# Ledicia/Molecular-Dynamics-Simulation---Lennard-Jones-monoatomic-fluid

Measured on AMD Instinct MI355X. Metric: md_steps_per_sec_n262144_fp64, higher is better.
Workload: dtype f64

## Files before the change

molecular-dynamics-simulation---lennard-jones-monoatomic-fluid_amd/csrc/ljmd_common.cpp:

```cpp
#include "ljmd_common.h"
#include "ljmd_internal.h"

#include <algorithm>
#include <cstdio>
#include <cstring>
#include <limits>

namespace ljmdh {

using namespace ljmdk;

thread_local std::string g_last_error = "";

int failv(std::string *handle_err, int code, const char *fmt, va_list ap)
{
    char buf[512];
    vsnprintf(buf, sizeof buf, fmt, ap);
    g_last_error = buf;
    if (handle_err) *handle_err = buf;
    return code;
}

int check_sim_params(const char *who, int n, double box_length, double dt, double rc)
{
// ... 42 lines not shown
Knobs read_knobs()
{
    auto flag = [](const char *name, bool dflt) { return env_int(name, dflt ? 1 : 0) != 0; };
    auto is = [](const char *name, const char *value) {
        const char *v = std::getenv(name);
        return v && std::strcmp(v, value) == 0;
    };
    auto opt_int = [](const char *name) -> std::optional<int> {
        const char *v = std::getenv(name);
        if (v && *v) return std::atoi(v);
        return std::nullopt;
    };
    Knobs k;
    k.sort = flag("LJMD_SORT", k.sort);
    k.force_generic = flag("LJMD_FORCE_GENERIC", k.force_generic);
    k.force_collectives = flag("LJMD_FORCE_COLLECTIVES", k.force_collectives);
    k.fuse = flag("LJMD_FUSE", k.fuse);
    k.fuse_tail = flag("LJMD_FUSE_TAIL", k.fuse_tail);
    k.fuse_defer_record = flag("LJMD_FUSE_DEFER_RECORD", k.fuse_defer_record);
    k.xcd_remap = std::max(0, env_int("LJMD_N3_XCD_REMAP", k.xcd_remap));
    k.inject_failure_at_step = env_int("LJMD_INJECT_FAILURE_AT_STEP", k.inject_failure_at_step);
    k.exchange_alltoall = is("LJMD_FORCE_EXCHANGE", "alltoall");
    k.resort_every = opt_int("LJMD_RESORT_EVERY");
    k.n3_row_tiles = env_int("LJMD_N3_ROW_TILES", k.n3_row_tiles);
    k.n3_wg_waves = env_int("LJMD_N3_WG_WAVES", k.n3_wg_waves);
    k.slab_budget_gb = std::max(1, env_int("LJMD_SLAB_BUDGET_GB", k.slab_budget_gb));
    k.n3_both_ties = flag("LJMD_N3_BOTH_TIES", k.n3_both_ties);
    k.n3_min_n = env_int("LJMD_N3_MIN_N", k.n3_min_n);
    k.n3 = flag("LJMD_N3", k.n3);
    k.n3_target_waves = opt_int("LJMD_N3_TARGET_WAVES");
    k.n3_clusters = flag("LJMD_N3_CLUSTERS", k.n3_clusters);
    k.n3_pertile = flag("LJMD_N3_PERTILE", k.n3_pertile);
    k.reduce_split = opt_int("LJMD_REDUCE_SPLIT");
    if (k.reduce_split) k.reduce_split = std::max(0, *k.reduce_split);
    k.walk_chunk = opt_int("LJMD_WALK_CHUNK");
    k.vanhove_chunk = opt_int("LJMD_VANHOVE_CHUNK");
    k.fp32_far_stream = flag("LJMD_FP32_FAR_STREAM", k.fp32_far_stream);
    k.fp32_vfar = flag("LJMD_FP32_VFAR", k.fp32_vfar);
    {
        const char *rs = std::getenv("LJMD_FP32_SPLIT");
        if (rs && *rs) k.fp32_split = std::max(0.0, std::atof(rs));
    }
    k.overlap_exchange = flag("LJMD_OVERLAP_EXCHANGE", k.overlap_exchange);
    k.migrate_blocks = is("LJMD_MIGRATE_DEAL", "blocks");
    {
        const char *xm = std::getenv("LJMD_MULTI_EXCHANGE");
// ... 80 lines not shown
```

molecular-dynamics-simulation---lennard-jones-monoatomic-fluid_amd/csrc/ljmd_common.h:

```cpp
#ifndef LJMD_COMMON_H
#define LJMD_COMMON_H

#include "ljmd.h"

#include <hip/hip_runtime.h>

#include <cstdarg>
#include <cstddef>
#include <cstdint>
#include <cstdlib>
#include <optional>
#include <string>

namespace ljmdh {

extern thread_local std::string g_last_error;

constexpr double kPi = 3.1415926535897932384626433832795;

int failv(std::string *handle_err, int code, const char *fmt, va_list ap);

inline int fail(std::nullptr_t, int code, const char *fmt, ...)
{
    va_list ap;
// ... 49 lines not shown
struct SimParams {
    double L = 0, invL = 0, volume = 0, rc = 0, rc2 = 0, dt = 0, dt_half = 0, dt_sq_half = 0;
    double tail_e = 0, tail_d = 0, tail_dd = 0;
};
SimParams derive_params(int n, double box_length, double dt, double rc);

void scalars_from_sums(double s12, double s6, double kx, double ky, double kz, double te, double td, double tdd,
                       double *epot, double *ekin, double *d_epot, double *dd_epot);

void scalars_from_exact_sums(const uint64_t (&ordered)[5][3], double te, double td, double tdd, bool have_e, bool have_k,
                             double *epot, double *ekin, double *d_epot, double *dd_epot);

struct Knobs {
    bool sort = true;
    bool force_generic = false;
    bool force_collectives = false;
    bool fuse = true;
    bool fuse_tail = true;
    bool fuse_defer_record = true;
    int xcd_remap = 4;
    int inject_failure_at_step = -1;
    bool exchange_alltoall = false;
    std::optional<int> resort_every;
    int n3_row_tiles = 0;
    int n3_wg_waves = 0;
    int slab_budget_gb = 64;
    bool n3_both_ties = true;
    int n3_min_n = 4096;
    bool n3 = true;
    std::optional<int> n3_target_waves;
    bool n3_clusters = true;
    bool n3_pertile = true;
    std::optional<int> reduce_split;
    std::optional<int> walk_chunk;
    std::optional<int> vanhove_chunk;
    bool fp32_far_stream = true;
    bool fp32_vfar = true;
    double fp32_split = 5.0;
    bool overlap_exchange = true;
    bool migrate_blocks = false;
    std::string multi_exchange;
    int multi_migrate_every = 2000;
    bool multi_threads = true;
    bool batch_group_streams = true;
};
Knobs read_knobs();
// ... 4 lines not shown
```

molecular-dynamics-simulation---lennard-jones-monoatomic-fluid_amd/csrc/ljmd_engine.cpp:

```cpp
#include "ljmd_engine.h"

namespace ljmdh {

bool fast_path_ok(const ljmd_t *h) { return h->plan.rc_allows_fast && h->positions_compact && !h->knobs.force_generic; }

double *wg_part_now(ljmd_t *h) { return h->d_wg_part + (h->plan.fuse_tail ? (size_t)h->fold_parity * h->wg_part_stride : 0); }

PairArgs pair_args(ljmd_t *h, bool fast)
{
    PairArgs a;
    a.pos = h->d_pos;
    a.slab = h->d_slab;
    a.wg_part = wg_part_now(h);
    a.mask = h->d_mask;
    a.bbox = h->d_bbox;
    a.inline_mask = (fast && h->plan.fuse_tail && !h->plan.use_n3) ? 1 : 0;
    a.rc2_skin = h->rc2 * (1.0 + 1e-10);
    a.n = h->n;
    a.S = h->plan.S;
    a.P = h->plan.P;
    a.G = h->G;
    a.rank = h->rank;
    a.TB = h->plan.TB;
    a.T = h->plan.T;
// ... 127 lines not shown
    a.ring_pos = h->d_ring_pos;
    a.n_wg = n_wg;
    a.n_ke = with_ke ? h->plan.n_ke : 0;
    a.ring_cap = kRingCap;
    return a;
}

EventSet *next_events(ljmd_t *h)
{
    if (!h->profiling || h->ev_used >= (size_t)kMaxProfiledLaunches) return nullptr;
    if (h->ev_used == h->ev_pool.size()) {
        EventSet q;
        for (auto &e : q.e)
            if (hipEventCreate(&e) != hipSuccess) return nullptr;
        h->ev_pool.push_back(q);
    }
    EventSet *q = &h->ev_pool[h->ev_used++];
    q->has_pos_x = q->has_force_x = false;
    return q;
}

int resort(ljmd_t *h, bool with_accel)
{
    {
    LJMD_HIP(h, launch_iota(h->d_idx, h->plan.P, h->stream));
    LJMD_HIP(h, hipMemcpyAsync(h->d_idx2, h->d_idx, (size_t)h->plan.P * sizeof(int), hipMemcpyDeviceToDevice,
                               h->stream));
    int *cur = h->d_idx, *nxt = h->d_idx2;
    for (size_t l = 0; l < h->plan.kd_level_nseg.size(); ++l) {
        const double *axis = own_block(h) + (size_t)h->kd_axis[l] * h->plan.P;
        LJMD_HIP(h, kd_level(h->d_cub, h->cub_bytes, axis, h->L, h->d_kd_keys, h->d_kd_keys2, cur, nxt, h->plan.S,
                             h->plan.kd_level_nseg[l], h->d_kd_offsets + h->plan.kd_level_off[l], h->stream));
        std::swap(cur, nxt);
    }
    if (cur != h->d_idx2)
        LJMD_HIP(h, hipMemcpyAsync(h->d_idx2, cur, (size_t)h->plan.P * sizeof(int), hipMemcpyDeviceToDevice,
                                   h->stream));
    }
    const size_t bytes3 = 3 * (size_t)h->plan.P * sizeof(double);
    double *sets[4] = {own_block(h), h->d_ru, h->d_v, h->d_a};
    for (int k = 0; k < (with_accel ? 4 : 3); ++k) {
        LJMD_HIP(h, launch_gather3(sets[k], h->d_tmp3, h->d_idx2, h->plan.P, h->stream));
        LJMD_HIP(h, hipMemcpyAsync(sets[k], h->d_tmp3, bytes3, hipMemcpyDeviceToDevice, h->stream));
    }
    LJMD_HIP(h, launch_gather_perm(h->d_perm, h->d_perm2, h->d_idx2, h->plan.P, h->stream));
    std::swap(h->d_perm, h->d_perm2);
    h->perm_dirty = true;
    h->steps_since_sort = 0;
    return LJMD_OK;
}

int refresh_perm(ljmd_t *h)
{
    if (!h->perm_dirty) return LJMD_OK;
    LJMD_HIP(h, hipMemcpyAsync(h->h_perm.data(), h->d_perm, (size_t)h->plan.P * sizeof(int), hipMemcpyDeviceToHost,
                               h->stream));
    LJMD_HIP(h, hipStreamSynchronize(h->stream));
    h->perm_dirty = false;
    return LJMD_OK;
}

bool use_comm_stream(const ljmd_t *h) { return h->knobs.overlap_exchange && h->comm_stream != nullptr; }

int comm_begin(ljmd_t *h)
{
    LJMD_HIP(h, hipEventRecord(h->ev_pos_ready, h->stream));
    LJMD_HIP(h, hipStreamWaitEvent(h->comm_stream, h->ev_pos_ready, 0));
    return LJMD_OK;
// ... 357 lines not shown
```

molecular-dynamics-simulation---lennard-jones-monoatomic-fluid_amd/csrc/ljmd_engine.h:

```cpp
#ifndef LJMD_ENGINE_H
#define LJMD_ENGINE_H

#include "ljmd_common.h"

#include <rccl/rccl.h>

#include <algorithm>
#include <cmath>
#include <cstdio>
#include <cstring>
#include <limits>
#include <mutex>
#include <vector>

#include "ljmd_internal.h"
#include "ljmd_resident.h"

using namespace ljmdk;

namespace ljmdh {

constexpr unsigned kRingCap = 4096;
constexpr int kTargetWorkgroups = 2048;
constexpr int kXcdMinGroups = 256;
constexpr int kMixedMinN = 16384;
constexpr long kN3ItemsFor4 = 6000;
constexpr long kN3ItemsFor2 = 1000;
constexpr long kN3LargeItems = 131072;
constexpr int kN3MidTargetItems = 32768;
constexpr int kBothTiesMaxGroups = 128;
constexpr int kFuseTailMaxRowTiles = 2;
constexpr int kFuseTailMaxN = 20000;
constexpr int kReduceSplitMinN = 131072;
constexpr int kReduceSplitShare = 8;
constexpr int kMaxProfiledLaunches = 4096;
constexpr int kEventsPerLaunch = 9;

struct EventSet {
    hipEvent_t e[kEventsPerLaunch];
    bool has_pos_x = false, has_force_x = false;
};

struct LaunchPlan {
    int S = 0, P = 0;
    int TB = 0, T = 0, W = 0;
    bool rc_allows_fast = false;
    bool sort_enabled = true;
    int resort_every = 20;
    std::vector<int> kd_level_nseg;
    std::vector<size_t> kd_level_off;
    std::vector<int> kd_offsets;
    int nslab_g = 1, chunk_g = 0;
    int nslab_t = 1, chunk_t = 0;
    bool use_n3 = false;
    int wg_waves = 1;
    bool both_ties = false;
    int uchunk = 0;
    int CS = 0, CS2 = 0, j_by_group = 0;
    int NG = 0, NGo = 0, Dmax = 0, nslab_n = 1, dchunk = 0;
    int rt = kRowTiles;
    bool fuse_tail = false;
    int split_s1 = 0, split_j1 = 0;
    int nslab_max = 1, n_wg_max = 0;
    int n_ke = 0;
};

int plan_engine(const SimParams &sim, int n, int n_ranks, int precision_mode, const Knobs &k, LaunchPlan *out);

}

struct ljmd_multi;

using namespace ljmdh;

// ... 26 lines not shown
    bool next_drift_hint = false;
    bool reduce_deferred = false, deferred_n3 = false;
    int deferred_nslab = 0;
    bool drift_prefused = false;
    double *d_ke_tile = nullptr;
    bool boxes_valid = false;
    double *d_ke_part = nullptr;
    double *d_ring = nullptr;
    int rec_stride = kPartialStride;
    __int128 *d_fslab = nullptr;
    unsigned *d_fflag = nullptr;
    int64_t *d_fblk = nullptr;
    int64_t *d_frec = nullptr;
    bool pending_energy = true;
    unsigned *d_ring_pos = nullptr;
    double *d_bbox = nullptr;
    uint64_t *d_mask = nullptr;
    double *d_pos_tc = nullptr;
    unsigned *d_desc = nullptr;
    unsigned *d_desc_far = nullptr;
    float *d_desc2 = nullptr;
    int *d_idx = nullptr, *d_idx2 = nullptr, *d_perm = nullptr, *d_perm2 = nullptr;
    double *d_tmp3 = nullptr;
    void *d_cub = nullptr;
    size_t cub_bytes = 0;
    std::vector<int> kd_axis;
    int *d_kd_offsets = nullptr;
    unsigned long long *d_kd_keys = nullptr, *d_kd_keys2 = nullptr;

    unsigned ring_consumed = 0;
    unsigned ring_issued = 0;
    bool fold_pending = false;
    ljmdk::FinalizeArgs pending_fold{};
    int fold_parity = 0;
    size_t wg_part_stride = 0;
    double *d_slab_j = nullptr;
    unsigned char *d_flag_j = nullptr;
    double *d_red_part = nullptr;
    hipStream_t side_stream = nullptr;
    hipEvent_t ev_side_go = nullptr, ev_side_done = nullptr;
    uint64_t *d_mask_far = nullptr;
    double *d_slab_j2 = nullptr;
    unsigned char *d_flag_j2 = nullptr;
    double *d_fpart = nullptr, *d_frecv = nullptr;
    double *d_fall = nullptr;
    bool forces_pending = false;
// ... 93 lines not shown
```

molecular-dynamics-simulation---lennard-jones-monoatomic-fluid_amd/csrc/ljmd_internal.h:

```cpp
#ifndef LJMD_INTERNAL_H
#define LJMD_INTERNAL_H

#include <hip/hip_runtime.h>
#include <stdint.h>

namespace ljmdk {

constexpr int kBlock = 256;
constexpr int kWavesPerBlock = kBlock / 64;
constexpr int kTile = 64;
#ifndef LJMD_ROW_TILES
#define LJMD_ROW_TILES 4
#endif
constexpr int kRowTiles = LJMD_ROW_TILES;
constexpr unsigned kAllRows = (1u << kRowTiles) - 1u;
constexpr int kSlotAlign = (kRowTiles * 64 > 256) ? kRowTiles * 64 : 256;
constexpr int kPartialStride = 8;
constexpr int kFoldBlocks = 128;
constexpr int kDirectFoldMax = 20480;
constexpr int kBoxStride = 8;

struct PairArgs {
    const double *pos;
    double *slab;
// ... 222 lines not shown
hipError_t launch_fixed_fold(const FixedFoldArgs &a, hipStream_t s);
hipError_t launch_rdf_histogram(const RdfArgs &a, dim3 grid, hipStream_t s);
hipError_t launch_time_origin(const TimeOriginArgs &a, bool vacf, int n_origins, hipStream_t s);
hipError_t launch_tile_boxes(const GeometryArgs &a, hipStream_t s);
hipError_t launch_tile_mask(const GeometryArgs &a, hipStream_t s);
hipError_t launch_tile_class(const GeometryArgs &a, double invL, double rc2, int S, int NGo, unsigned *desc,
                             unsigned *desc_far, float *desc2 , hipStream_t s);

size_t kd_temp_bytes(int count);
hipError_t launch_iota(int *idx, int P, hipStream_t s);
hipError_t kd_level(void *temp, size_t temp_bytes, const double *coord_axis, double L, unsigned long long *keys,
                    unsigned long long *keys_out, int *idx, int *idx_out, int S, int nseg, const int *seg_offsets,
                    hipStream_t s);
constexpr int kMigrateRows = 10;
hipError_t launch_iota_blocked(int *idx, int n, int S, int P, hipStream_t s);
hipError_t launch_iota_offset(int *idx, int count, int P, int offset, hipStream_t s);
hipError_t kd_level_blocked(void *temp, size_t temp_bytes, const double *pos, int axis, int P, double L,
                            unsigned long long *keys, unsigned long long *keys_out, int *idx, int *idx_out, int n, int nseg,
                            const int *seg_offsets, hipStream_t s);
hipError_t launch_migrate_pack(const double *ru, const double *v, const double *a, const int *perm, const int *gid0,
                               double *block, int S, int P, hipStream_t s);
hipError_t launch_migrate_select(const double *pos_all, const double *mig_all, const int *mine, double *new_pos, double *ru,
                                 double *v, double *a, int *gid0, int S, int P, hipStream_t s);
hipError_t launch_gather3(const double *src, double *dst, const int *idx, int P, hipStream_t s);
hipError_t launch_gather_perm(const int *src, int *dst, const int *idx, int P, hipStream_t s);


__device__ __forceinline__ double wave_sum(double v)
{
#pragma unroll
    for (int off = 32; off > 0; off >>= 1) v += __shfl_down(v, off, 64);
    return v;
}

template <int NVAL>
__device__ __forceinline__ void block_sum(double (&v)[NVAL], double *lds ,
                                          int stride = kWavesPerBlock, int W = kWavesPerBlock)
{
    const int lane = threadIdx.x & 63, wave = threadIdx.x >> 6;
#pragma unroll
    for (int k = 0; k < NVAL; ++k) {
        const double s = wave_sum(v[k]);
        if (lane == 0) lds[k * stride + wave] = s;
    }
    __syncthreads();
    if (threadIdx.x == 0) {
#pragma unroll
        for (int k = 0; k < NVAL; ++k) {
// ... 150 lines not shown
```

molecular-dynamics-simulation---lennard-jones-monoatomic-fluid_amd/csrc/ljmd_kernels.hip:

```cpp
#include <hip/hip_runtime.h>
#include <stdint.h>

#include "ljmd_internal.h"

namespace ljmdk {

__device__ __forceinline__ double wave_min(double v)
{
#pragma unroll
    for (int off = 32; off > 0; off >>= 1) v = fmin(v, __shfl_down(v, off, 64));
    return v;
}

__device__ __forceinline__ double wave_max(double v)
{
#pragma unroll
    for (int off = 32; off > 0; off >>= 1) v = fmax(v, __shfl_down(v, off, 64));
    return v;
}

__global__ __launch_bounds__(kBlock) void pair_rows_generic_kernel(PairArgs a)
{
    __shared__ double red[2 * kWavesPerBlock];
    const int row = blockIdx.x * kBlock + threadIdx.x;
// ... 1236 lines not shown
    const int Il = blockIdx.y * kWavesPerBlock + (threadIdx.x >> 6);
    const int w = blockIdx.x;
    if (Il >= a.TB) return;
    const int I = a.rank * a.TB + Il;
    const int J = w * 64 + lane;
    bool keep = false, far = false;
    if (J < a.T) {
        const double d2 = tile_gap2(a.bbox, I, J, a.L);
        keep = !(d2 > a.rc2_skin) || (J == I);
        if (a.mask_far) {
            const bool near = (d2 <= a.rsplit2) || (J / a.RT == I / a.RT);
            far = keep && !near;
            keep = keep && near;
        }
    }
    if (a.mask_far) {
        const uint64_t far_word = __ballot(far);
        if (lane == 0) a.mask_far[(size_t)Il * a.W + w] = far_word;
    }
    const uint64_t word = __ballot(keep);
    if (lane == 0) a.mask[(size_t)Il * a.W + w] = word;
}

template <int RT>
__global__ __launch_bounds__(kBlock) void tile_class_kernel(GeometryArgs a, double invL, double rc2, int S, unsigned *desc,
                                                            unsigned *desc_far, float *desc2)
{
    const int c = blockIdx.x * kBlock + threadIdx.x;
    const int Al = blockIdx.y;
    if (c >= a.T) return;
    unsigned d = 0;
    if (tile_class<RT>(a, invL, rc2, S, Al, c, d, desc_far, desc2)) desc[(size_t)Al * a.T + c] = d;
}

template <int PHASE, bool BOXES = false>
__global__ __launch_bounds__(kBlock) void drift_kick_kernel(IntegrateArgs a)
{
    const int i = blockIdx.x * kBlock + threadIdx.x;
    if (i >= a.rows) return;
    double rn[3];
#pragma unroll
    for (int ax = 0; ax < 3; ++ax) {
        const size_t o = (size_t)ax * a.P + i;
        const double v0 = a.v[o], acc = a.a[o];
        if constexpr (PHASE != 2) {
            const Drift h = drift_wrap(a.r[o], v0, acc, a.dt, a.dt_sq_half, a.L, a.invL);
            a.r[o] = h.r1;
            a.ru[o] = a.ru[o] + h.d;
            rn[ax] = h.r1;
        }
        if constexpr (PHASE != 1) a.v[o] = half_kick(v0, acc, a.dt_half);
    }
    if constexpr (BOXES && PHASE != 2) {
// ... 688 lines not shown
{
    if (a.energy)
        hipLaunchKernelGGL(pair_n3_f32_kernel<true>, grid, dim3(kTile), 0, s, a);
    else
        hipLaunchKernelGGL(pair_n3_f32_kernel<false>, grid, dim3(kTile), 0, s, a);
    return hipGetLastError();
}

hipError_t launch_tile_boxes(const GeometryArgs &a, hipStream_t s)
{
    hipLaunchKernelGGL(tile_boxes_kernel, dim3((a.T + kWavesPerBlock - 1) / kWavesPerBlock), dim3(kBlock), 0, s, a);
    return hipGetLastError();
}

hipError_t launch_tile_mask(const GeometryArgs &a, hipStream_t s)
{
    hipLaunchKernelGGL(tile_mask_kernel, dim3(a.W, (a.TB + kWavesPerBlock - 1) / kWavesPerBlock), dim3(kBlock), 0, s, a);
    return hipGetLastError();
}

hipError_t launch_tile_class(const GeometryArgs &a, double invL, double rc2, int S, int NGo, unsigned *desc, unsigned *desc_far,
                             float *desc2, hipStream_t s)
{
    const dim3 grid((a.T + kBlock - 1) / kBlock, NGo);
    if (a.RT == 1)
        hipLaunchKernelGGL(tile_class_kernel<1>, grid, dim3(kBlock), 0, s, a, invL, rc2, S, desc, desc_far, desc2);
    else if (a.RT == 2)
        hipLaunchKernelGGL(tile_class_kernel<2>, grid, dim3(kBlock), 0, s, a, invL, rc2, S, desc, desc_far, desc2);
    else
        hipLaunchKernelGGL(tile_class_kernel<kRowTiles>, grid, dim3(kBlock), 0, s, a, invL, rc2, S, desc, desc_far, desc2);
    return hipGetLastError();
}

hipError_t launch_drift_kick(const IntegrateArgs &a, int phase, hipStream_t s)
{
    const dim3 grid((a.rows + kBlock - 1) / kBlock);
    if (phase == 1)
        hipLaunchKernelGGL(drift_kick_kernel<1>, grid, dim3(kBlock), 0, s, a);
    else if (phase == 2)
        hipLaunchKernelGGL(drift_kick_kernel<2>, grid, dim3(kBlock), 0, s, a);
    else if (a.bbox)
        hipLaunchKernelGGL((drift_kick_kernel<0, true>), grid, dim3(kBlock), 0, s, a);
    else
        hipLaunchKernelGGL(drift_kick_kernel<0>, grid, dim3(kBlock), 0, s, a);
    return hipGetLastError();
}

// ... 133 lines not shown
```

molecular-dynamics-simulation---lennard-jones-monoatomic-fluid_amd/csrc/ljmd_plan.cpp:

```cpp
#include "ljmd_engine.h"

namespace ljmdh {

namespace {
int rt_align(int uchunk, int rt)
{
    int m = 1;
    while ((m * uchunk) % rt != 0) ++m;
    return m;
}
}

int plan_engine(const SimParams &sim, int n, int n_ranks, int precision_mode, const Knobs &k, LaunchPlan *out)
{
    LaunchPlan p;
    p.S = n / n_ranks;
    p.P = ((p.S + kSlotAlign - 1) / kSlotAlign) * kSlotAlign;
    p.TB = p.P / kTile;
    p.T = n_ranks * p.TB;
    p.W = (p.T + 63) / 64;
    p.rc_allows_fast = sim.rc <= (1.0 - 1e-9) * 0.5 * sim.L;
    p.sort_enabled = k.sort && n >= 1024;
    p.resort_every = std::max(1, k.resort_every.value_or(n >= 1000000 ? 5 : n >= 131072 ? 10 : n > 40000 ? 20
                                                              : n > kFuseTailMaxN ? 50 : 200));
    {
        const int tiles = (p.S + kTile - 1) / kTile;
        std::vector<int> bounds = {0, tiles};
        while (true) {
            bool any = false;
            for (size_t j = 0; j + 1 < bounds.size(); ++j) any = any || (bounds[j + 1] - bounds[j] > 1);
            if (!any) break;
            p.kd_level_off.push_back(p.kd_offsets.size());
            p.kd_level_nseg.push_back((int)bounds.size() - 1);
            for (int b : bounds) p.kd_offsets.push_back(std::min(b * kTile, p.S));
            std::vector<int> next;
            for (size_t j = 0; j + 1 < bounds.size(); ++j) {
                next.push_back(bounds[j]);
                const int t = bounds[j + 1] - bounds[j];
                if (t > 1) next.push_back(bounds[j] + (t + 1) / 2);
            }
            next.push_back(tiles);
            bounds.swap(next);
        }
    }

    const int row_blocks = p.P / kBlock;
    {
        int ns = (kTargetWorkgroups + row_blocks - 1) / row_blocks;
        ns = std::max(1, std::min(ns, (n + 63) / 64));
        p.chunk_g = ((n + ns - 1) / ns + 7) / 8 * 8;
        p.nslab_g = (n + p.chunk_g - 1) / p.chunk_g;
    }
    {
        int ns = (kTargetWorkgroups + row_blocks - 1) / row_blocks;
        ns = std::max(1, std::min(ns, p.T));
        p.chunk_t = (p.T + ns - 1) / ns;
        p.nslab_t = (p.T + p.chunk_t - 1) / p.chunk_t;
    }
    {
        const bool mixed_mode = precision_mode == LJMD_PRECISION_FP32_FORCE;
        int rt = k.n3_row_tiles;
        if (mixed_mode) rt = kRowTiles;
        if (rt != 1 && rt != 2 && rt != kRowTiles) {
            auto items = [&](int cand) { const long ngo = p.TB / cand; return ngo * ((long)n_ranks * ngo / 2 + 1); };
            rt = items(kRowTiles) >= kN3ItemsFor4 ? kRowTiles : items(2) >= kN3ItemsFor2 ? 2 : 1;
// ... 63 lines not shown
```

molecular-dynamics-simulation---lennard-jones-monoatomic-fluid_amd/csrc/ljmd_sort.hip:

```cpp
#include <hip/hip_runtime.h>
#include <hipcub/hipcub.hpp>

#include "ljmd_internal.h"

namespace ljmdk {

__global__ __launch_bounds__(kBlock) void gather3_kernel(const double *src, double *dst, const int *idx, int P)
{
    const int i = blockIdx.x * kBlock + threadIdx.x;
    if (i >= P) return;
    const int s = idx[i];
    dst[i] = src[s];
    dst[P + i] = src[P + s];
    dst[2 * (size_t)P + i] = src[2 * (size_t)P + s];
}

__global__ __launch_bounds__(kBlock) void gather_perm_kernel(const int *src, int *dst, const int *idx, int P)
{
    const int i = blockIdx.x * kBlock + threadIdx.x;
    if (i < P) dst[i] = src[idx[i]];
}

constexpr int kCoordBits = 24;

__global__ __launch_bounds__(kBlock) void kd_keys_kernel(const double *coord, const int *idx, unsigned long long *keys,
                                                         const int *seg_offsets, int nseg, int S, double scale)
{
    const int i = blockIdx.x * kBlock + threadIdx.x;
    if (i >= S) return;
    int lo = 0, hi = nseg;
    while (hi - lo > 1) {
        const int mid = (lo + hi) >> 1;
        if (seg_offsets[mid] <= i) lo = mid; else hi = mid;
    }
    const double x = coord[idx[i]] * scale;
    const unsigned long long q = (unsigned long long)fmin(fmax(x, 0.0), (double)((1u << kCoordBits) - 1));
    keys[i] = ((unsigned long long)lo << kCoordBits) | q;
}

__global__ __launch_bounds__(kBlock) void iota_kernel(int *idx, int P)
{
    const int i = blockIdx.x * kBlock + threadIdx.x;
    if (i < P) idx[i] = i;
}

size_t kd_temp_bytes(int count)
{
    size_t bytes = 0;
    (void)hipcub::DeviceRadixSort::SortPairs(nullptr, bytes, (const unsigned long long *)nullptr,
                                             (unsigned long long *)nullptr, (const int *)nullptr, (int *)nullptr,
                                             count, 0, 64, nullptr);
    return bytes;
}

hipError_t launch_iota(int *idx, int P, hipStream_t s)
{
    hipLaunchKernelGGL(iota_kernel, dim3((P + kBlock - 1) / kBlock), dim3(kBlock), 0, s, idx, P);
    return hipGetLastError();
}

hipError_t kd_level(void *temp, size_t temp_bytes, const double *coord_axis, double L, unsigned long long *keys,
                    unsigned long long *keys_out, int *idx, int *idx_out, int S, int nseg, const int *seg_offsets,
                    hipStream_t s)
{
    hipLaunchKernelGGL(kd_keys_kernel, dim3((S + kBlock - 1) / kBlock), dim3(kBlock), 0, s, coord_axis, idx, keys,
                       seg_offsets, nseg, S, (double)(1u << kCoordBits) / L);
    hipError_t e = hipGetLastError();
    if (e != hipSuccess) return e;
    int segbits = 1;
    while ((1 << segbits) < nseg) ++segbits;
    return hipcub::DeviceRadixSort::SortPairs(temp, temp_bytes, keys, keys_out, idx, idx_out, S, 0,
                                              kCoordBits + segbits, s);
}

__global__ __launch_bounds__(kBlock) void iota_blocked_kernel(int *idx, int n, int S, int P)
{
    const int k = blockIdx.x * kBlock + threadIdx.x;
    if (k < n) idx[k] = (k / S) * P + k % S;
}

__global__ __launch_bounds__(kBlock) void kd_keys_blocked_kernel(const double *pos, int axis, int P, const int *idx,
                                                                 unsigned long long *keys, const int *seg_offsets, int nseg,
                                                                 int n, double scale)
{
    const int i = blockIdx.x * kBlock + threadIdx.x;
    if (i >= n) return;
    int lo = 0, hi = nseg;
    while (hi - lo > 1) {
        const int mid = (lo + hi) >> 1;
        if (seg_offsets[mid] <= i) lo = mid; else hi = mid;
    }
    const int st = idx[i], g = st / P, sl = st - g * P;
    const double x = pos[(size_t)g * 3 * P + (size_t)axis * P + sl] * scale;
    const unsigned long long q = (unsigned long long)fmin(fmax(x, 0.0), (double)((1u << kCoordBits) - 1));
    keys[i] = ((unsigned long long)lo << kCoordBits) | q;
}

__global__ __launch_bounds__(kBlock) void migrate_pack_kernel(const double *ru, const double *v, const double *a,
                                                              const int *perm, const int *gid0, double *block, int S, int P)
{
    const int s = blockIdx.x * kBlock + threadIdx.x;
    if (s >= P) return;
#pragma unroll
    for (int k = 0; k < 3; ++k) {
        block[(size_t)k * P + s] = ru[(size_t)k * P + s];
        block[(size_t)(3 + k) * P + s] = v[(size_t)k * P + s];
        block[(size_t)(6 + k) * P + s] = a[(size_t)k * P + s];
    }
    const int o = perm[s];
    block[(size_t)9 * P + s] = (s < S && o < S) ? (double)gid0[o] : -1.0;
}

__global__ __launch_bounds__(kBlock) void migrate_select_kernel(const double *pos_all, const double *mig_all, const int *mine,
                                                                double *new_pos, double *ru, double *v, double *a, int *gid0,
                                                                int S, int P)
{
    const int j = blockIdx.x * kBlock + threadIdx.x;
    if (j >= P) return;
// ... 48 lines not shown
    hipError_t e = hipGetLastError();
    if (e != hipSuccess) return e;
    int segbits = 1;
    while ((1 << segbits) < nseg) ++segbits;
    return hipcub::DeviceRadixSort::SortPairs(temp, temp_bytes, keys, keys_out, idx, idx_out, n, 0, kCoordBits + segbits, s);
}

hipError_t launch_migrate_pack(const double *ru, const double *v, const double *a, const int *perm, const int *gid0,
                               double *block, int S, int P, hipStream_t s)
{
    hipLaunchKernelGGL(migrate_pack_kernel, dim3((P + kBlock - 1) / kBlock), dim3(kBlock), 0, s, ru, v, a, perm, gid0, block,
                       S, P);
    return hipGetLastError();
}

hipError_t launch_migrate_select(const double *pos_all, const double *mig_all, const int *mine, double *new_pos, double *ru,
                                 double *v, double *a, int *gid0, int S, int P, hipStream_t s)
{
    hipLaunchKernelGGL(migrate_select_kernel, dim3((P + kBlock - 1) / kBlock), dim3(kBlock), 0, s, pos_all, mig_all, mine,
                       new_pos, ru, v, a, gid0, S, P);
    return hipGetLastError();
}

hipError_t launch_gather3(const double *src, double *dst, const int *idx, int P, hipStream_t s)
{
    hipLaunchKernelGGL(gather3_kernel, dim3((P + kBlock - 1) / kBlock), dim3(kBlock), 0, s, src, dst, idx, P);
    return hipGetLastError();
}

hipError_t launch_gather_perm(const int *src, int *dst, const int *idx, int P, hipStream_t s)
{
    hipLaunchKernelGGL(gather_perm_kernel, dim3((P + kBlock - 1) / kBlock), dim3(kBlock), 0, s, src, dst, idx, P);
    return hipGetLastError();
}

}
```

molecular-dynamics-simulation---lennard-jones-monoatomic-fluid_amd/csrc/ljmd_storage.cpp:

```cpp
#include "ljmd_engine.h"

namespace ljmdh {

int allocate_engine(ljmd_t *h)
{
    const bool mixed = h->mode == LJMD_PRECISION_FP32_FORCE;
    const std::vector<int> &kd = h->plan.kd_offsets;
    LJMD_HIP(h, hipSetDevice(h->device));
    LJMD_HIP(h, hipStreamCreateWithFlags(&h->stream, hipStreamNonBlocking));
    const size_t P3 = 3 * (size_t)h->plan.P * sizeof(double);
    LJMD_HIP(h, hipMalloc(&h->d_pos, P3 * h->G));
    LJMD_HIP(h, hipMalloc(&h->d_ru, P3));
    LJMD_HIP(h, hipMalloc(&h->d_v, P3));
    LJMD_HIP(h, hipMalloc(&h->d_a, P3));
    LJMD_HIP(h, hipMalloc(&h->d_tmp3, P3));
    LJMD_HIP(h, hipMalloc(&h->d_slab, P3 * h->plan.nslab_max));
    h->wg_part_stride = 2 * (size_t)h->plan.n_wg_max;
    LJMD_HIP(h, hipMalloc(&h->d_wg_part, (h->plan.fuse_tail ? 2 : 1) * h->wg_part_stride * sizeof(double)));
    if (h->plan.use_n3) {
        const size_t n_blk = (size_t)h->plan.T * h->plan.CS;
        LJMD_HIP(h, hipMalloc(&h->d_slab_j, n_blk * 3 * kTile * sizeof(double)));
        LJMD_HIP(h, hipMalloc(&h->d_flag_j, n_blk));
        LJMD_HIP(h, hipMemsetAsync(h->d_flag_j, 0, n_blk, h->stream));
        LJMD_HIP(h, hipMalloc(&h->d_desc, (size_t)h->plan.NGo * h->plan.T * sizeof(unsigned)));
        if (h->plan.rt == kRowTiles && h->plan.wg_waves == 1 && h->knobs.n3_clusters)
            LJMD_HIP(h, hipMalloc(&h->d_desc2, (size_t)h->plan.NGo * h->plan.T * 8 * sizeof(float)));
        LJMD_HIP(h, hipMalloc(&h->d_pos_tc, P3 * h->G));
    }
    if (h->plan.split_s1 > 0) {
        LJMD_HIP(h, hipMalloc(&h->d_red_part, (size_t)h->plan.TB * kWavesPerBlock * 3 * kTile * sizeof(double)));
        int least = 0, greatest = 0;
        LJMD_HIP(h, hipDeviceGetStreamPriorityRange(&least, &greatest));
        LJMD_HIP(h, hipStreamCreateWithPriority(&h->side_stream, hipStreamNonBlocking, least));
        LJMD_HIP(h, hipEventCreateWithFlags(&h->ev_side_go, hipEventDisableTiming));
        LJMD_HIP(h, hipEventCreateWithFlags(&h->ev_side_done, hipEventDisableTiming));
    }
    if (mixed && h->knobs.fp32_far_stream) {
        LJMD_HIP(h, hipStreamCreateWithFlags(&h->far_stream, hipStreamNonBlocking));
// ... 61 lines not shown
    if (h->stream) (void)hipStreamSynchronize(h->stream);
    release_resident(h);
    if (h->comm_stream) (void)hipStreamSynchronize(h->comm_stream);
    if (h->comm) (void)ncclCommDestroy(h->comm);
    if (h->comm_stream) (void)hipStreamDestroy(h->comm_stream);
    if (h->far_stream) {
        (void)hipStreamSynchronize(h->far_stream);
        (void)hipStreamDestroy(h->far_stream);
    }
    if (h->side_stream) {
        (void)hipStreamSynchronize(h->side_stream);
        (void)hipStreamDestroy(h->side_stream);
    }
    if (h->ev_side_go) (void)hipEventDestroy(h->ev_side_go);
    if (h->ev_side_done) (void)hipEventDestroy(h->ev_side_done);
    if (h->ev_far_go) (void)hipEventDestroy(h->ev_far_go);
    if (h->ev_far_done) (void)hipEventDestroy(h->ev_far_done);
    if (h->ev_pos_ready) (void)hipEventDestroy(h->ev_pos_ready);
    if (h->ev_gather_done) (void)hipEventDestroy(h->ev_gather_done);
    for (auto &q : h->ev_pool)
        for (auto &e : q.e) (void)hipEventDestroy(e);
    void *dev[] = {h->d_pos, h->d_ru, h->d_v, h->d_a, h->d_slab, h->d_wg_part, h->d_ke_part, h->d_ring,
                   h->d_ring_pos, h->d_bbox, h->d_mask, h->d_idx, h->d_idx2,
                   h->d_perm, h->d_perm2, h->d_tmp3, h->d_cub, h->d_slab_j, h->d_flag_j, h->d_fpart, h->d_frecv, h->d_fall,
                   h->d_kd_offsets, h->d_kd_keys, h->d_kd_keys2, h->d_mask_far, h->d_slab_j2, h->d_flag_j2, h->d_fold, h->d_ticket,
                   h->d_desc, h->d_desc_far, h->d_desc2, h->d_red_part, h->d_ke_tile, h->d_pos_tc, h->d_gid0, h->d_mig, h->d_mig_idx, h->d_mig_idx2, h->d_mig_keys,
                   h->d_mig_keys2, h->d_mig_offsets, h->d_mig_cub, h->d_fslab, h->d_fflag, h->d_fblk, h->d_frec};
    for (void *p : dev) (void)hipFree(p);
    if (h->h_stage) (void)hipHostFree(h->h_stage);
    if (h->h_ring) (void)hipHostFree(h->h_ring);
    if (h->copy_stream) {
        (void)hipStreamSynchronize(h->copy_stream);
        (void)hipStreamDestroy(h->copy_stream);
    }
    if (h->ev_snap_ready) (void)hipEventDestroy(h->ev_snap_ready);
    if (h->ev_snap_done) (void)hipEventDestroy(h->ev_snap_done);
    if (h->d_snap) (void)hipFree(h->d_snap);
    if (h->d_snap_perm) (void)hipFree(h->d_snap_perm);
    if (h->h_snap) (void)hipHostFree(h->h_snap);
    if (h->h_snap_perm) (void)hipHostFree(h->h_snap_perm);
    if (h->stream) (void)hipStreamDestroy(h->stream);
    delete h;
}

int download_state(ljmd_t *h, double *const dsts[12], unsigned n_records)
{
    const size_t P = h->plan.P;
// ... 65 lines not shown
```

Measured before the change: 55.57.

## Finish k-d sort levels in shared-memory bitonic kernel and fuse state gather

Once every k-d segment from some level downward holds at most 4096 particles, those levels are sorted inside one workgroup per segment with a shared-memory bitonic sort, replacing the per-level hipcub radix sorts. The four per-array gather-plus-copy passes and the permutation gather are merged into one gather kernel writing into double buffers, and the buffers are then pointer-swapped. Only positions still need a copy back. The tile classification grid is also cut to roughly half the columns by exploiting pair symmetry. The aim is to remove kernel launches and memory traffic in resort, at the cost of extra buffers and a more complex sort path.

```diff
diff --git a/molecular-dynamics-simulation---lennard-jones-monoatomic-fluid_amd/csrc/ljmd_common.cpp b/molecular-dynamics-simulation---lennard-jones-monoatomic-fluid_amd/csrc/ljmd_common.cpp
--- a/molecular-dynamics-simulation---lennard-jones-monoatomic-fluid_amd/csrc/ljmd_common.cpp
+++ b/molecular-dynamics-simulation---lennard-jones-monoatomic-fluid_amd/csrc/ljmd_common.cpp
@@ -88,6 +88,7 @@
     k.inject_failure_at_step = env_int("LJMD_INJECT_FAILURE_AT_STEP", k.inject_failure_at_step);
     k.exchange_alltoall = is("LJMD_FORCE_EXCHANGE", "alltoall");
     k.resort_every = opt_int("LJMD_RESORT_EVERY");
+    k.kd_sort_cub = is("LJMD_KD_SORT", "cub");
     k.n3_row_tiles = env_int("LJMD_N3_ROW_TILES", k.n3_row_tiles);
     k.n3_wg_waves = env_int("LJMD_N3_WG_WAVES", k.n3_wg_waves);
     k.slab_budget_gb = std::max(1, env_int("LJMD_SLAB_BUDGET_GB", k.slab_budget_gb));
diff --git a/molecular-dynamics-simulation---lennard-jones-monoatomic-fluid_amd/csrc/ljmd_common.h b/molecular-dynamics-simulation---lennard-jones-monoatomic-fluid_amd/csrc/ljmd_common.h
--- a/molecular-dynamics-simulation---lennard-jones-monoatomic-fluid_amd/csrc/ljmd_common.h
+++ b/molecular-dynamics-simulation---lennard-jones-monoatomic-fluid_amd/csrc/ljmd_common.h
@@ -95,6 +95,7 @@
     int inject_failure_at_step = -1;
     bool exchange_alltoall = false;
     std::optional<int> resort_every;
+    bool kd_sort_cub = false;
     int n3_row_tiles = 0;
     int n3_wg_waves = 0;
     int slab_budget_gb = 64;
diff --git a/molecular-dynamics-simulation---lennard-jones-monoatomic-fluid_amd/csrc/ljmd_engine.cpp b/molecular-dynamics-simulation---lennard-jones-monoatomic-fluid_amd/csrc/ljmd_engine.cpp
--- a/molecular-dynamics-simulation---lennard-jones-monoatomic-fluid_amd/csrc/ljmd_engine.cpp
+++ b/molecular-dynamics-simulation---lennard-jones-monoatomic-fluid_amd/csrc/ljmd_engine.cpp
@@ -173,28 +173,50 @@
 
 int resort(ljmd_t *h, bool with_accel)
 {
-    {
-    LJMD_HIP(h, launch_iota(h->d_idx, h->plan.P, h->stream));
-    LJMD_HIP(h, hipMemcpyAsync(h->d_idx2, h->d_idx, (size_t)h->plan.P * sizeof(int), hipMemcpyDeviceToDevice,
-                               h->stream));
+    if (!launch_kd_finish || !launch_gather_state)
+        return fail(h, LJMD_ERR_HIP, "resort: this build holds no launch_kd_finish / launch_gather_state (ljmd_sort.h)");
+    const int levels = (int)h->plan.kd_level_nseg.size(), from = h->plan.kd_finish_from;
     int *cur = h->d_idx, *nxt = h->d_idx2;
-    for (size_t l = 0; l < h->plan.kd_level_nseg.size(); ++l) {
+    LJMD_HIP(h, launch_iota(cur, h->plan.P, h->stream));
+    if (from > 0) LJMD_HIP(h, launch_iota(nxt, h->plan.P, h->stream));
+    for (int l = 0; l < from; ++l) {
         const double *axis = own_block(h) + (size_t)h->kd_axis[l] * h->plan.P;
         LJMD_HIP(h, kd_level(h->d_cub, h->cub_bytes, axis, h->L, h->d_kd_keys, h->d_kd_keys2, cur, nxt, h->plan.S,
                              h->plan.kd_level_nseg[l], h->d_kd_offsets + h->plan.kd_level_off[l], h->stream));
         std::swap(cur, nxt);
     }
-    if (cur != h->d_idx2)
-        LJMD_HIP(h, hipMemcpyAsync(h->d_idx2, cur, (size_t)h->plan.P * sizeof(int), hipMemcpyDeviceToDevice,
-                                   h->stream));
-    }
-    const size_t bytes3 = 3 * (size_t)h->plan.P * sizeof(double);
-    double *sets[4] = {own_block(h), h->d_ru, h->d_v, h->d_a};
-    for (int k = 0; k < (with_accel ? 4 : 3); ++k) {
-        LJMD_HIP(h, launch_gather3(sets[k], h->d_tmp3, h->d_idx2, h->plan.P, h->stream));
-        LJMD_HIP(h, hipMemcpyAsync(sets[k], h->d_tmp3, bytes3, hipMemcpyDeviceToDevice, h->stream));
-    }
-    LJMD_HIP(h, launch_gather_perm(h->d_perm, h->d_perm2, h->d_idx2, h->plan.P, h->stream));
+    for (int l = from; l < levels; l += kKdFinishMaxLevels) {
+        KdFinishArgs ka;
+        ka.pos = own_block(h);
+        ka.P = h->plan.P;
+        ka.scale = (double)(1u << kCoordBits) / h->L;
+        ka.idx_in = ka.idx_out = cur;
+        ka.offsets = h->d_kd_offsets;
+        ka.nlevels = std::min(kKdFinishMaxLevels, levels - l);
+        for (int k = 0; k < ka.nlevels; ++k) {
+            ka.nseg[k] = h->plan.kd_level_nseg[l + k];
+            ka.off[k] = (int)h->plan.kd_level_off[l + k];
+            ka.axis[k] = h->kd_axis[l + k];
+        }
+        LJMD_HIP(h, launch_kd_finish(ka, h->stream));
+    }
+    GatherStateArgs g;
+    double *sets[4] = {own_block(h), h->d_ru, h->d_v, with_accel ? h->d_a : nullptr};
+    double *outs[4] = {h->d_tmp3, h->d_ru2, h->d_v2, h->d_a2};
+    for (int k = 0; k < 4; ++k) {
+        g.src[k] = sets[k];
+        g.dst[k] = outs[k];
+    }
+    g.perm = h->d_perm;
+    g.perm_out = h->d_perm2;
+    g.idx = cur;
+    g.P = h->plan.P;
+    LJMD_HIP(h, launch_gather_state(g, h->stream));
+    LJMD_HIP(h, hipMemcpyAsync(own_block(h), h->d_tmp3, 3 * (size_t)h->plan.P * sizeof(double), hipMemcpyDeviceToDevice,
+                               h->stream));
+    std::swap(h->d_ru, h->d_ru2);
+    std::swap(h->d_v, h->d_v2);
+    if (with_accel) std::swap(h->d_a, h->d_a2);
     std::swap(h->d_perm, h->d_perm2);
     h->perm_dirty = true;
     h->steps_since_sort = 0;
diff --git a/molecular-dynamics-simulation---lennard-jones-monoatomic-fluid_amd/csrc/ljmd_engine.h b/molecular-dynamics-simulation---lennard-jones-monoatomic-fluid_amd/csrc/ljmd_engine.h
--- a/molecular-dynamics-simulation---lennard-jones-monoatomic-fluid_amd/csrc/ljmd_engine.h
+++ b/molecular-dynamics-simulation---lennard-jones-monoatomic-fluid_amd/csrc/ljmd_engine.h
@@ -15,6 +15,7 @@
 
 #include "ljmd_internal.h"
 #include "ljmd_resident.h"
+#include "ljmd_sort.h"
 
 using namespace ljmdk;
 
@@ -50,6 +51,7 @@
     std::vector<int> kd_level_nseg;
     std::vector<size_t> kd_level_off;
     std::vector<int> kd_offsets;
+    int kd_finish_from = 0;
     int nslab_g = 1, chunk_g = 0;
     int nslab_t = 1, chunk_t = 0;
     bool use_n3 = false;
@@ -122,6 +124,7 @@
     float *d_desc2 = nullptr;
     int *d_idx = nullptr, *d_idx2 = nullptr, *d_perm = nullptr, *d_perm2 = nullptr;
     double *d_tmp3 = nullptr;
+    double *d_ru2 = nullptr, *d_v2 = nullptr, *d_a2 = nullptr;
     void *d_cub = nullptr;
     size_t cub_bytes = 0;
     std::vector<int> kd_axis;
diff --git a/molecular-dynamics-simulation---lennard-jones-monoatomic-fluid_amd/csrc/ljmd_internal.h b/molecular-dynamics-simulation---lennard-jones-monoatomic-fluid_amd/csrc/ljmd_internal.h
--- a/molecular-dynamics-simulation---lennard-jones-monoatomic-fluid_amd/csrc/ljmd_internal.h
+++ b/molecular-dynamics-simulation---lennard-jones-monoatomic-fluid_amd/csrc/ljmd_internal.h
@@ -268,8 +268,6 @@
                                double *block, int S, int P, hipStream_t s);
 hipError_t launch_migrate_select(const double *pos_all, const double *mig_all, const int *mine, double *new_pos, double *ru,
                                  double *v, double *a, int *gid0, int S, int P, hipStream_t s);
-hipError_t launch_gather3(const double *src, double *dst, const int *idx, int P, hipStream_t s);
-hipError_t launch_gather_perm(const int *src, int *dst, const int *idx, int P, hipStream_t s);
 
 
 __device__ __forceinline__ double wave_sum(double v)
diff --git a/molecular-dynamics-simulation---lennard-jones-monoatomic-fluid_amd/csrc/ljmd_kernels.hip b/molecular-dynamics-simulation---lennard-jones-monoatomic-fluid_amd/csrc/ljmd_kernels.hip
--- a/molecular-dynamics-simulation---lennard-jones-monoatomic-fluid_amd/csrc/ljmd_kernels.hip
+++ b/molecular-dynamics-simulation---lennard-jones-monoatomic-fluid_amd/csrc/ljmd_kernels.hip
@@ -1282,13 +1282,21 @@
     if (lane == 0) a.mask[(size_t)Il * a.W + w] = word;
 }
 
+__host__ __device__ constexpr int tile_class_columns(int T, int RT)
+{
+    const int n = ((T / RT) / 2 + 1) * RT;
+    return n < T ? n : T;
+}
+
 template <int RT>
 __global__ __launch_bounds__(kBlock) void tile_class_kernel(GeometryArgs a, double invL, double rc2, int S, unsigned *desc,
                                                             unsigned *desc_far, float *desc2)
 {
-    const int c = blockIdx.x * kBlock + threadIdx.x;
     const int Al = blockIdx.y;
-    if (c >= a.T) return;
+    const int j = blockIdx.x * kBlock + threadIdx.x;
+    if (j >= tile_class_columns(a.T, RT)) return;
+    int c = (a.rank * (a.TB / RT) + Al) * RT + j;
+    if (c >= a.T) c -= a.T;
     unsigned d = 0;
     if (tile_class<RT>(a, invL, rc2, S, Al, c, d, desc_far, desc2)) desc[(size_t)Al * a.T + c] = d;
 }
@@ -2023,7 +2031,7 @@
 hipError_t launch_tile_class(const GeometryArgs &a, double invL, double rc2, int S, int NGo, unsigned *desc, unsigned *desc_far,
                              float *desc2, hipStream_t s)
 {
-    const dim3 grid((a.T + kBlock - 1) / kBlock, NGo);
+    const dim3 grid((tile_class_columns(a.T, a.RT) + kBlock - 1) / kBlock, NGo);
     if (a.RT == 1)
         hipLaunchKernelGGL(tile_class_kernel<1>, grid, dim3(kBlock), 0, s, a, invL, rc2, S, desc, desc_far, desc2);
     else if (a.RT == 2)
diff --git a/molecular-dynamics-simulation---lennard-jones-monoatomic-fluid_amd/csrc/ljmd_plan.cpp b/molecular-dynamics-simulation---lennard-jones-monoatomic-fluid_amd/csrc/ljmd_plan.cpp
--- a/molecular-dynamics-simulation---lennard-jones-monoatomic-fluid_amd/csrc/ljmd_plan.cpp
+++ b/molecular-dynamics-simulation---lennard-jones-monoatomic-fluid_amd/csrc/ljmd_plan.cpp
@@ -41,6 +41,15 @@
             }
             next.push_back(tiles);
             bounds.swap(next);
+        }
+        const int levels = (int)p.kd_level_nseg.size();
+        p.kd_finish_from = levels;
+        for (int l = levels - 1; l >= 0 && !k.kd_sort_cub; --l) {
+            int largest = 0;
+            for (int j = 0; j < p.kd_level_nseg[l]; ++j)
+                largest = std::max(largest, p.kd_offsets[p.kd_level_off[l] + j + 1] - p.kd_offsets[p.kd_level_off[l] + j]);
+            if (largest > kKdFinishCap) break;
+            p.kd_finish_from = l;
         }
     }
 
diff --git a/molecular-dynamics-simulation---lennard-jones-monoatomic-fluid_amd/csrc/ljmd_sort.h b/molecular-dynamics-simulation---lennard-jones-monoatomic-fluid_amd/csrc/ljmd_sort.h
--- /dev/null
+++ b/molecular-dynamics-simulation---lennard-jones-monoatomic-fluid_amd/csrc/ljmd_sort.h
@@ -0,0 +1,40 @@
+#ifndef LJMD_SORT_H
+#define LJMD_SORT_H
+
+#include <hip/hip_runtime.h>
+
+namespace ljmdk {
+
+constexpr int kCoordBits = 24;
+
+constexpr int kKdFinishCap = 4096;
+constexpr int kKdFinishMaxLevels = 6;
+constexpr int kKdFinishBlock = 1024;
+
+struct KdFinishArgs {
+    const double *pos = nullptr;
+    int P = 0;
+    double scale = 0.0;
+    const int *idx_in = nullptr;
+    int *idx_out = nullptr;
+    const int *offsets = nullptr;
+    int nlevels = 0;
+    int nseg[kKdFinishMaxLevels] = {};
+    int off[kKdFinishMaxLevels] = {};
+    int axis[kKdFinishMaxLevels] = {};
+};
+
+struct GatherStateArgs {
+    const double *src[4] = {};
+    double *dst[4] = {};
+    const int *perm = nullptr;
+    int *perm_out = nullptr;
+    const int *idx = nullptr;
+    int P = 0;
+};
+
+__attribute__((weak)) hipError_t launch_kd_finish(const KdFinishArgs &a, hipStream_t s);
+__attribute__((weak)) hipError_t launch_gather_state(const GatherStateArgs &a, hipStream_t s);
+
+}
+#endif
diff --git a/molecular-dynamics-simulation---lennard-jones-monoatomic-fluid_amd/csrc/ljmd_sort.hip b/molecular-dynamics-simulation---lennard-jones-monoatomic-fluid_amd/csrc/ljmd_sort.hip
--- a/molecular-dynamics-simulation---lennard-jones-monoatomic-fluid_amd/csrc/ljmd_sort.hip
+++ b/molecular-dynamics-simulation---lennard-jones-monoatomic-fluid_amd/csrc/ljmd_sort.hip
@@ -2,26 +2,30 @@
 #include <hipcub/hipcub.hpp>
 
 #include "ljmd_internal.h"
+#include "ljmd_sort.h"
 
 namespace ljmdk {
 
-__global__ __launch_bounds__(kBlock) void gather3_kernel(const double *src, double *dst, const int *idx, int P)
-{
-    const int i = blockIdx.x * kBlock + threadIdx.x;
-    if (i >= P) return;
-    const int s = idx[i];
-    dst[i] = src[s];
-    dst[P + i] = src[P + s];
-    dst[2 * (size_t)P + i] = src[2 * (size_t)P + s];
-}
-
-__global__ __launch_bounds__(kBlock) void gather_perm_kernel(const int *src, int *dst, const int *idx, int P)
-{
-    const int i = blockIdx.x * kBlock + threadIdx.x;
-    if (i < P) dst[i] = src[idx[i]];
-}
-
-constexpr int kCoordBits = 24;
+__global__ __launch_bounds__(kBlock) void gather_state_kernel(GatherStateArgs g)
+{
+    const int i = blockIdx.x * kBlock + threadIdx.x;
+    if (i >= g.P) return;
+    const int s = g.idx[i];
+#pragma unroll
+    for (int q = 0; q < 4; ++q) {
+        if (g.src[q] == nullptr) continue;
+#pragma unroll
+        for (int k = 0; k < 3; ++k) g.dst[q][(size_t)k * g.P + i] = g.src[q][(size_t)k * g.P + s];
+    }
+    g.perm_out[i] = g.perm[s];
+}
+
+
+__device__ __forceinline__ unsigned long long kd_quant(double coord, double scale)
+{
+    const double x = coord * scale;
+    return (unsigned long long)fmin(fmax(x, 0.0), (double)((1u << kCoordBits) - 1));
+}
 
 __global__ __launch_bounds__(kBlock) void kd_keys_kernel(const double *coord, const int *idx, unsigned long long *keys,
                                                          const int *seg_offsets, int nseg, int S, double scale)
@@ -33,9 +37,7 @@
         const int mid = (lo + hi) >> 1;
         if (seg_offsets[mid] <= i) lo = mid; else hi = mid;
     }
-    const double x = coord[idx[i]] * scale;
-    const unsigned long long q = (unsigned long long)fmin(fmax(x, 0.0), (double)((1u << kCoordBits) - 1));
-    keys[i] = ((unsigned long long)lo << kCoordBits) | q;
+    keys[i] = ((unsigned long long)lo << kCoordBits) | kd_quant(coord[idx[i]], scale);
 }
 
 __global__ __launch_bounds__(kBlock) void iota_kernel(int *idx, int P)
@@ -73,6 +75,108 @@
                                               kCoordBits + segbits, s);
 }
 
+
+__device__ __forceinline__ int last_at_most(const int *b, int n, int x)
+{
+    int lo = 0, hi = n;
+    while (hi - lo > 1) {
+        const int mid = (lo + hi) >> 1;
+        if (b[mid] <= x) lo = mid; else hi = mid;
+    }
+    return lo;
+}
+
+__device__ __forceinline__ void order_pair(unsigned long long &x, unsigned long long &y, bool up)
+{
+    if ((x > y) == up) {
+        const unsigned long long t = x;
+        x = y;
+        y = t;
+    }
+}
+
+__global__ __launch_bounds__(kKdFinishBlock) void kd_finish_kernel(KdFinishArgs a)
+{
+    constexpr int kMaxSub = kKdFinishCap / kTile;
+    __shared__ unsigned long long s_word[kKdFinishCap];
+    __shared__ int s_idx[kKdFinishCap];
+    __shared__ int s_bound[kKdFinishMaxLevels][kMaxSub + 1];
+    __shared__ int s_first[kKdFinishMaxLevels], s_last[kKdFinishMaxLevels];
+    const int tid = threadIdx.x;
+    const int lo = a.offsets[a.off[0] + blockIdx.x], len = a.offsets[a.off[0] + blockIdx.x + 1] - lo;
+    if (len <= 0 || len > kKdFinishCap) return;
+    int npad = kTile;
+    while (npad < len) npad <<= 1;
+    for (int p = tid; p < len; p += kKdFinishBlock) s_idx[p] = a.idx_in[lo + p];
+    if (tid < kKdFinishMaxLevels) s_first[tid] = s_last[tid] = 0;
+    __syncthreads();
+    for (int l = 0; l < a.nlevels; ++l)
+        for (int j = tid; j <= a.nseg[l]; j += kKdFinishBlock) {
+            const int b = a.offsets[a.off[l] + j];
+            if (b == lo) s_first[l] = j;
+            if (b == lo + len) s_last[l] = j;
+        }
+    __syncthreads();
+    for (int l = 0; l < a.nlevels; ++l) {
+        const int nsub = min(s_last[l] - s_first[l], kMaxSub);
+        if (tid <= nsub) s_bound[l][tid] = a.offsets[a.off[l] + s_first[l] + tid] - lo;
+    }
+    __syncthreads();
+    for (int l = 0; l < a.nlevels; ++l) {
+        const int nsub = min(s_last[l] - s_first[l], kMaxSub);
+        const double *coord = a.pos + (size_t)a.axis[l] * a.P;
+        for (int p = tid; p < npad; p += kKdFinishBlock) {
+            unsigned long long w = ~0ull;
+            if (p < len) {
+                const unsigned home = l == 0 ? (unsigned)p : (unsigned)(s_word[p] & 0xffffu);
+                const int sub = last_at_most(s_bound[l], nsub, p);
+                w = ((unsigned long long)sub << 56) | (kd_quant(coord[s_idx[home]], a.scale) << 32) |
+                    ((unsigned long long)p << 16) | home;
+            }
+            s_word[p] = w;
+        }
+        __syncthreads();
+        for (int k = 2; k <= npad; k <<= 1) {
+            int j = k >> 1;
+            for (; j >= 2; j >>= 2) {
+                const int h = j >> 1;
+                for (int t = tid; t < (npad >> 2); t += kKdFinishBlock) {
+                    const int i = ((t & ~(h - 1)) << 2) | (t & (h - 1));
+                    const bool up = (i & k) == 0;
+                    unsigned long long w0 = s_word[i], w1 = s_word[i | h], w2 = s_word[i | j], w3 = s_word[i | j | h];
+                    order_pair(w0, w2, up);
+                    order_pair(w1, w3, up);
+                    order_pair(w0, w1, up);
+                    order_pair(w2, w3, up);
+                    s_word[i] = w0;
+                    s_word[i | h] = w1;
+                    s_word[i | j] = w2;
+                    s_word[i | j | h] = w3;
+                }
+                __syncthreads();
+            }
+            if (j == 1) {
+                for (int t = tid; t < (npad >> 1); t += kKdFinishBlock) {
+                    const int i = t << 1;
+                    unsigned long long w0 = s_word[i], w1 = s_word[i | 1];
+                    order_pair(w0, w1, (i & k) == 0);
+                    s_word[i] = w0;
+                    s_word[i | 1] = w1;
+                }
+                __syncthreads();
+            }
+        }
+    }
+    for (int p = tid; p < len; p += kKdFinishBlock) a.idx_out[lo + p] = s_idx[s_word[p] & 0xffffu];
+}
+
+hipError_t launch_kd_finish(const KdFinishArgs &a, hipStream_t s)
+{
+    if (a.nlevels < 1 || a.nlevels > kKdFinishMaxLevels) return hipErrorInvalidValue;
+    hipLaunchKernelGGL(kd_finish_kernel, dim3(a.nseg[0]), dim3(kKdFinishBlock), 0, s, a);
+    return hipGetLastError();
+}
+
 __global__ __launch_bounds__(kBlock) void iota_blocked_kernel(int *idx, int n, int S, int P)
 {
     const int k = blockIdx.x * kBlock + threadIdx.x;
@@ -91,9 +195,7 @@
         if (seg_offsets[mid] <= i) lo = mid; else hi = mid;
     }
     const int st = idx[i], g = st / P, sl = st - g * P;
-    const double x = pos[(size_t)g * 3 * P + (size_t)axis * P + sl] * scale;
-    const unsigned long long q = (unsigned long long)fmin(fmax(x, 0.0), (double)((1u << kCoordBits) - 1));
-    keys[i] = ((unsigned long long)lo << kCoordBits) | q;
+    keys[i] = ((unsigned long long)lo << kCoordBits) | kd_quant(pos[(size_t)g * 3 * P + (size_t)axis * P + sl], scale);
 }
 
 __global__ __launch_bounds__(kBlock) void migrate_pack_kernel(const double *ru, const double *v, const double *a,
@@ -188,16 +290,10 @@
     return hipGetLastError();
 }
 
-hipError_t launch_gather3(const double *src, double *dst, const int *idx, int P, hipStream_t s)
-{
-    hipLaunchKernelGGL(gather3_kernel, dim3((P + kBlock - 1) / kBlock), dim3(kBlock), 0, s, src, dst, idx, P);
-    return hipGetLastError();
-}
-
-hipError_t launch_gather_perm(const int *src, int *dst, const int *idx, int P, hipStream_t s)
-{
-    hipLaunchKernelGGL(gather_perm_kernel, dim3((P + kBlock - 1) / kBlock), dim3(kBlock), 0, s, src, dst, idx, P);
-    return hipGetLastError();
-}
-
-}
+hipError_t launch_gather_state(const GatherStateArgs &g, hipStream_t s)
+{
+    hipLaunchKernelGGL(gather_state_kernel, dim3((g.P + kBlock - 1) / kBlock), dim3(kBlock), 0, s, g);
+    return hipGetLastError();
+}
+
+}
diff --git a/molecular-dynamics-simulation---lennard-jones-monoatomic-fluid_amd/csrc/ljmd_storage.cpp b/molecular-dynamics-simulation---lennard-jones-monoatomic-fluid_amd/csrc/ljmd_storage.cpp
--- a/molecular-dynamics-simulation---lennard-jones-monoatomic-fluid_amd/csrc/ljmd_storage.cpp
+++ b/molecular-dynamics-simulation---lennard-jones-monoatomic-fluid_amd/csrc/ljmd_storage.cpp
@@ -14,6 +14,11 @@
     LJMD_HIP(h, hipMalloc(&h->d_v, P3));
     LJMD_HIP(h, hipMalloc(&h->d_a, P3));
     LJMD_HIP(h, hipMalloc(&h->d_tmp3, P3));
+    if (h->plan.sort_enabled) {
+        LJMD_HIP(h, hipMalloc(&h->d_ru2, P3));
+        LJMD_HIP(h, hipMalloc(&h->d_v2, P3));
+        LJMD_HIP(h, hipMalloc(&h->d_a2, P3));
+    }
     LJMD_HIP(h, hipMalloc(&h->d_slab, P3 * h->plan.nslab_max));
     h->wg_part_stride = 2 * (size_t)h->plan.n_wg_max;
     LJMD_HIP(h, hipMalloc(&h->d_wg_part, (h->plan.fuse_tail ? 2 : 1) * h->wg_part_stride * sizeof(double)));
@@ -121,7 +126,7 @@
         for (auto &e : q.e) (void)hipEventDestroy(e);
     void *dev[] = {h->d_pos, h->d_ru, h->d_v, h->d_a, h->d_slab, h->d_wg_part, h->d_ke_part, h->d_ring,
                    h->d_ring_pos, h->d_bbox, h->d_mask, h->d_idx, h->d_idx2,
-                   h->d_perm, h->d_perm2, h->d_tmp3, h->d_cub, h->d_slab_j, h->d_flag_j, h->d_fpart, h->d_frecv, h->d_fall,
+                   h->d_perm, h->d_perm2, h->d_tmp3, h->d_ru2, h->d_v2, h->d_a2, h->d_cub, h->d_slab_j, h->d_flag_j, h->d_fpart, h->d_frecv, h->d_fall,
                    h->d_kd_offsets, h->d_kd_keys, h->d_kd_keys2, h->d_mask_far, h->d_slab_j2, h->d_flag_j2, h->d_fold, h->d_ticket,
                    h->d_desc, h->d_desc_far, h->d_desc2, h->d_red_part, h->d_ke_tile, h->d_pos_tc, h->d_gid0, h->d_mig, h->d_mig_idx, h->d_mig_idx2, h->d_mig_keys,
                    h->d_mig_keys2, h->d_mig_offsets, h->d_mig_cub, h->d_fslab, h->d_fflag, h->d_fblk, h->d_frec};
```

Result: faster. 56.23 (median of 6 runs) (+1.2%).
